# visinf/style-seqcvae

Hardware: AMD Instinct MI355X
Metric: captions/sec (train step) (higher is better)
Workload: dtype f32; 1 GPU; C2 train step: fwd+bwd+allreduce+clip+SGD, B=64/GPU, R=36, F=2048, L=20 (T=21), Z=128, V=10000, E=1000, H=1200, A=768, SENTIMENT_VAE=1; global_batch=64, parallelism=dp1

## Files before the change

style-seqcvae_amd/csrc/gemm.hip:

```cpp
#include <stdio.h>
#include <stdlib.h>
#include <string.h>

#include <type_traits>

#include "ssc_common.h"
#include "ssc_debug.h"

typedef float f32x16 __attribute__((ext_vector_type(16)));

namespace {

constexpr int BM = 64, BN = 64, BK = 32;
constexpr int KC_LD = BK + 4;

struct KSeg {
  const float* A;
  const float* B;
  int lda, ldb, K, nsteps;
  int avec, bvec;
  const float* A16;
  const float* B16;
  int lda16, ldb16;
};
// ... 829 lines not shown
      SSC_X3B_MFMA(1, 1)
      SSC_X3B_MFMA(1, 0)
      SSC_X3B_MFMA(0, 1)
      SSC_X3B_MFMA(0, 0)
#undef SSC_X3B_MFMA
    }
  };

  for (int s = s_lo; s < s_hi; ++s) {
    compute();
    wait_loads();
    __syncthreads();
    if (s + 1 < s_hi) put_planes();
    advance();
    issue_loads();
    __syncthreads();
  }
  wait_loads();

  float* out = a.out + (size_t)z * a.slab_stride;
#pragma unroll
  for (int ni = 0; ni < 2; ++ni) {
    const int col = n0 + wn * 64 + ni * 32 + l31;
    if (col >= a.N) continue;
    const float bv = (a.bias != nullptr) ? a.bias[col] : 0.f;
#pragma unroll
    for (int mi = 0; mi < 2; ++mi) {
      const int rbase = m0 + wm * 64 + mi * 32 + 4 * half;
      int rr[16];
#pragma unroll
      for (int r = 0; r < 16; ++r) {
        rr[r] = min(rbase + (r & 3) + 8 * (r >> 2), Meff - 1);
        if (a.crows) rr[r] = a.crows[rr[r]];
      }
      float old[16];
      if (a.accumulate) {
#pragma unroll
        for (int r = 0; r < 16; ++r) old[r] = out[(size_t)rr[r] * a.ldo + col];
      } else {
#pragma unroll
        for (int r = 0; r < 16; ++r) old[r] = 0.f;
      }
#pragma unroll
      for (int r = 0; r < 16; ++r) {
        if (rbase + (r & 3) + 8 * (r >> 2) < Meff) out[(size_t)rr[r] * a.ldo + col] = acc[mi][ni][r] + bv + old[r];
      }
    }
  }
}


#ifdef SSC_X3W_STAMP
__device__ unsigned long long* g_stamp_ptr = nullptr;
__device__ int g_stamp_wg = -1;
#define SSC_STAMP(i)                                                                                  \
  do {                                                                                                \
    if (stamp_on && lane == 0 && (i) < 124) stamp_lds[(i)] = __builtin_readcyclecounter();           \
  } while (0)
constexpr int X3W_STAMP_BYTES = 2048;
#else
#define SSC_STAMP(i) do {} while (0)
constexpr int X3W_STAMP_BYTES = 0;
#endif
#ifdef SSC_X3W_AUDIT
constexpr int SSC_AUDIT_MEMBERS = 20;
__device__ long long g_audit[SSC_AUDIT_MEMBERS][SSC_MAX_SEG][2][2];
#define SSC_AUDIT_TOUCH(member, seg, op, off)                                       \
  do {                                                                              \
    atomicMin(&g_audit[(member)][(seg)][(op)][0], (long long)(off));                \
    atomicMax(&g_audit[(member)][(seg)][(op)][1], (long long)(off) + 16);           \
  } while (0)
#else
#define SSC_AUDIT_TOUCH(member, seg, op, off) do {} while (0)
#endif
template <int R> struct X3wPlane {
  static constexpr int MC_ROW_B = 2 * R + 64;
  static constexpr int KC_BYTES = R * PL_ROW_B, MC_BYTES = 32 * MC_ROW_B;
  static constexpr int BYTES = KC_BYTES > MC_BYTES ? KC_BYTES : MC_BYTES;
};
template <int TM, int TN> constexpr int x3w_lds_bytes() { return 2 * 3 * (X3wPlane<TM>::BYTES + X3wPlane<TN>::BYTES) + X3W_STAMP_BYTES; }
template <int TM, int TN> constexpr int x3w_lds_bytes_f16() { return 2 * 2 * (X3wPlane<TM>::BYTES + X3wPlane<TN>::BYTES) + X3W_STAMP_BYTES; }

struct KTnArgs;
template <bool A_KC, bool B_KC, bool KG, int TM, int TN, int PF, int NPW, bool F16 = false, class Args = KArgs>
__device__ __forceinline__ void x3w_body(const Args& a, const int blk_x, const int blk_y, const int blk_z, const int grid_x,
                                         const int grid_y, const int grid_z, const int thr) {
  static_assert((TM == 128 && TN == 128) || (TM == 64 && TN == 256), "unsupported tile");
  static_assert(PF == 1 || PF == 2, "prefetch depth");
  constexpr int UNR = 2;
  constexpr bool RL = TM == 128;
  static_assert(!KG || PF == 1, "the gather lists' own loads share the vector-memory counter");
  constexpr int NPL = F16 ? 2 : 3;
  constexpr int PLA = X3wPlane<TM>::BYTES, PLB = X3wPlane<TN>::BYTES, STAGE = NPL * (PLA + PLB);
  static_assert(TM * (TN + 4) * 4 <= 2 * STAGE, "the epilogue's C tile reuses the operand stages");
  constexpr int MCA = X3wPlane<TM>::MC_ROW_B, MCB = X3wPlane<TN>::MC_ROW_B;
  static_assert(NPW == 4 || NPW == 8, "producer waves");
  constexpr int NPT = 64 * NPW;
  constexpr int NTHR = 256 + NPT;
  constexpr int NA = TM * 8 / NPT, NB = TN * 8 / NPT;
  constexpr int QA = TM / 4, QB = TN / 4;
  auto kc_row = [&](int t, int u, int) __attribute__((always_inline)) -> int { return (t + NPT * u) >> 3; };
  extern __shared__ __attribute__((aligned(16))) unsigned char lds[];
  const int wave = thr >> 6;
  const bool producer = wave >= 4;
  const int tid = producer ? thr - 256 : thr;
  const int lane = tid & 63;
  int bx, by;
  const int Meff = (RL && a.mcount) ? min(a.M, *a.mcount) : a.M;
  const int gy_live = min(grid_y, (Meff + TM - 1) / TM);
  if (blk_y * grid_x + blk_x >= grid_x * gy_live) return;
  tile_order(blk_y * grid_x + blk_x, grid_x, gy_live, a.tile_gm, bx, by);
  const int n0 = bx * TN, m0 = by * TM, z = blk_z;
  if (m0 >= Meff) return;
  const int Kc = a.kcount ? max(0, min(a.seg[0].K, *a.kcount)) : 0;
  int steps_total = a.steps_total, steps_per_split = a.steps_per_split;
  if (a.kcount) {
    steps_total = (Kc + BK - 1) / BK;
    steps_per_split = (steps_total + grid_z - 1) / grid_z;
  }
  const int s_lo = z * steps_per_split;
  int s_hi = s_lo + steps_per_split;
  if (s_hi > steps_total) s_hi = steps_total;
  const int s_last = s_hi - 1;
  constexpr int CT_LD = TN + 4;
  float f16_sa = 1.f, f16_sb = 1.f;
  if constexpr (F16) {
    if (a.a_scale) f16_sa = *a.a_scale;
    if (a.b_scale) f16_sb = *a.b_scale;
  }
#ifdef SSC_X3W_STAMP
  const bool stamp_on = (int)blockIdx.x == g_stamp_wg && (wave == 0 || wave == 4);
  unsigned long long* stamp_lds = reinterpret_cast<unsigned long long*>(lds + 2 * STAGE) + (wave == 4 ? 0 : 128);
  if (stamp_on && lane == 0) { stamp_lds[126] = __builtin_readcyclecounter(); stamp_lds[127] = wall_clock64(); }
  const unsigned long long stamp_entry = wall_clock64();
#endif

  if (producer) {
    f32x4 ra[PF][NA], rb[PF][NB];
    unsigned oka[PF], okb[PF];
    bool fullk[PF];
    unsigned oa[NA], ob[NB];
    unsigned za[NA], zb[NB];
    int ia[2][NA], ib[2][NB];
    Cursor cur;
    int s_ld = s_lo;
    bool pa = false, pb = false;
    auto planes_of_segment = [&]() __attribute__((always_inline)) {
      if constexpr (F16) {
        const KSeg& sg = a.seg[cur.seg];
        pa = sg.A16 != nullptr; pb = sg.B16 != nullptr;
        if (pa) { cur.A = sg.A16; cur.lda = sg.lda16; }
        if (pb) { cur.B = sg.B16; cur.ldb = sg.ldb16; }
      }
    };
    auto base_ptrs = [&]() __attribute__((always_inline)) {
      const unsigned lda4 = (unsigned)cur.lda * 4u, ldb4 = (unsigned)cur.ldb * 4u;
#pragma unroll
      for (int u = 0; u < NA; ++u) {
        const int idx = tid + NPT * u;
        if constexpr (A_KC) {
          int r = min(m0 + kc_row(tid, u, NA), Meff - 1);
          if constexpr (RL) { if (a.arows) r = a.arows[r]; }
          za[u] = (unsigned)r * lda4;
          oa[u] = za[u] + 16u * (idx & 7);
        } else {
          za[u] = 4u * (unsigned)min(m0 + 4 * (idx % QA), Meff - 4);
          if constexpr (KG) {
            int kr = cur.k0 + idx / QA;
            kr = a.karows[min(kr, cur.K - 1)];
            oa[u] = (unsigned)kr;
          } else {
            oa[u] = (unsigned)(idx / QA) * lda4 + za[u];
          }
        }
      }
#pragma unroll
      for (int u = 0; u < NB; ++u) {
        const int idx = tid + NPT * u;
        if constexpr (B_KC) {
          zb[u] = (unsigned)min(n0 + kc_row(tid, u, NB), a.N - 1) * ldb4;
          ob[u] = zb[u] + 16u * (idx & 7);
        } else {
          zb[u] = 4u * (unsigned)min(n0 + 4 * (idx % QB), a.N - 4);
          if constexpr (KG) {
            int kr = cur.k0 + idx / QB;
            kr = a.kbrows[min(kr, cur.K - 1)];
            ob[u] = (unsigned)kr;
          } else {
            ob[u] = (unsigned)(idx / QB) * ldb4 + zb[u];
          }
        }
      }
    };
    auto prefetch_rows = [&](int buf) __attribute__((always_inline)) {
      if constexpr (KG) {
#pragma unroll
        for (int u = 0; u < NA; ++u) {
          const int kr = min(cur.k0 + BK + (tid + NPT * u) / QA, cur.K - 1);
          ia[buf][u] = a.karows[kr];
        }
#pragma unroll
        for (int u = 0; u < NB; ++u) {
          const int kr = min(cur.k0 + BK + (tid + NPT * u) / QB, cur.K - 1);
          ib[buf][u] = a.kbrows[kr];
        }
      }
    };
    auto step_ptrs = [&](int how, int buf) __attribute__((always_inline)) {
      if constexpr (KG) {
        if (how != 0) {
#pragma unroll
          for (int u = 0; u < NA; ++u) oa[u] = (unsigned)ia[buf][u];
#pragma unroll
          for (int u = 0; u < NB; ++u) ob[u] = (unsigned)ib[buf][u];
          prefetch_rows(buf ^ 1);
        }
      } else {
        if (how == 2) base_ptrs();
      }
    };
    auto issue_loads = [&](f32x4 (&xa)[NA], f32x4 (&xb)[NB], unsigned& ma, unsigned& mb, bool& full) __attribute__((always_inline)) {
      ma = pa ? 0x80000000u : 0u;
      mb = pb ? 0x80000000u : 0u;
      full = cur.k0 + BK <= cur.K;
      const float* sa = cur.A + (A_KC ? (size_t)cur.k0 : (KG ? (size_t)0 : (size_t)cur.k0 * cur.lda));
      const float* sb = cur.B + (B_KC ? (size_t)cur.k0 : (KG ? (size_t)0 : (size_t)cur.k0 * cur.ldb));
      unsigned ea[NA], eb[NB];
      const bool kc_in = cur.k0 + 4 * (tid & 7) < cur.K;
#pragma unroll
      for (int u = 0; u < NA; ++u) {
        const int idx = tid + NPT * u;
        if constexpr (A_KC) {
          ea[u] = (kc_in || pa) ? oa[u] : za[u];
          ma |= (kc_in ? 1u : 0u) << u;
        } else {
          const bool in = cur.k0 + idx / QA < cur.K;
          if constexpr (KG) ea[u] = __umul24(oa[u], (unsigned)cur.lda * 4u) + za[u];
          else ea[u] = in ? oa[u] : za[u];
          ma |= (in ? 1u : 0u) << u;
        }
      }
#pragma unroll
      for (int u = 0; u < NB; ++u) {
        const int idx = tid + NPT * u;
        if constexpr (B_KC) {
          eb[u] = (kc_in || pb) ? ob[u] : zb[u];
          mb |= (kc_in ? 1u : 0u) << u;
        } else {
          const bool in = cur.k0 + idx / QB < cur.K;
          if constexpr (KG) eb[u] = __umul24(ob[u], (unsigned)cur.ldb * 4u) + zb[u];
          else eb[u] = in ? ob[u] : zb[u];
          mb |= (in ? 1u : 0u) << u;
        }
      }
#ifdef SSC_X3W_AUDIT
#pragma unroll
      for (int u = 0; u < NA; ++u) SSC_AUDIT_TOUCH(a.member, cur.seg, 0, (reinterpret_cast<const char*>(sa) - reinterpret_cast<const char*>(cur.A)) + (long long)ea[u]);
#pragma unroll
      for (int u = 0; u < NB; ++u) SSC_AUDIT_TOUCH(a.member, cur.seg, 1, (reinterpret_cast<const char*>(sb) - reinterpret_cast<const char*>(cur.B)) + (long long)eb[u]);
#endif
#pragma unroll
      for (int u = 0; u < NA; ++u) asm volatile("global_load_dwordx4 %0, %1, %2" : "=&v"(xa[u]) : "v"(ea[u]), "s"(sa) : "memory");
#pragma unroll
      for (int u = 0; u < NB; ++u) asm volatile("global_load_dwordx4 %0, %1, %2" : "=&v"(xb[u]) : "v"(eb[u]), "s"(sb) : "memory");
    };
    auto pin = [&](f32x4 (&xa)[NA], f32x4 (&xb)[NB]) __attribute__((always_inline)) {
#pragma unroll
      for (int u = 0; u < NA; ++u) asm volatile("" : "+v"(xa[u])::"memory");
#pragma unroll
      for (int u = 0; u < NB; ++u) asm volatile("" : "+v"(xb[u])::"memory");
    };
    auto advance = [&](int buf) __attribute__((always_inline)) {
      const int how = cur.advance(a, s_ld >= s_last);
      s_ld = min(s_ld + 1, s_last);
      if (how == 2) planes_of_segment();
      step_ptrs(how, buf);
    };
    auto put_chunk = [&](unsigned char* p, int plane, f32x4 v, bool ok, float scale) __attribute__((always_inline)) {
      if (!ok) v = f32x4{0.f, 0.f, 0.f, 0.f};
      if constexpr (F16) {
        u32x2 hi, lo;
        v = v * scale;
        split4_f16(v, hi, lo);
        *reinterpret_cast<u32x2*>(p) = hi;
        *reinterpret_cast<u32x2*>(p + plane) = lo;
      } else {
        u32x2 hi, mid, lo;
// ... 299 lines not shown
        const float e[4] = {v.x, v.y, v.z, v.w};
#pragma unroll
        for (int q = 0; q < 4; ++q) {
          if (gcol + q < a.N) {
            const float r = e[q] + (a.bias ? a.bias[gcol + q] : 0.f) + (a.accumulate ? dst[q] : 0.f);
            dst[q] = r;
            if constexpr (std::is_same_v<Args, KTnArgs>) {
              if (a.out2) a.out2[(size_t)grow * a.ldo2 + gcol + q] = r;
            }
          }
        }
      }
    }
  }
#ifdef SSC_X3W_STAMP
  if (stamp_on && lane == 0) { stamp_lds[124] = __builtin_readcyclecounter(); stamp_lds[125] = wall_clock64(); }
  __syncthreads();
  if ((int)blockIdx.x == g_stamp_wg && thr < 256 && g_stamp_ptr)
    g_stamp_ptr[thr] = reinterpret_cast<const unsigned long long*>(lds + 2 * STAGE)[thr];
  if (g_stamp_wg == -2 && thr == 0 && g_stamp_ptr && blockIdx.x < 1024) {
    g_stamp_ptr[2 * blockIdx.x] = stamp_entry;
    g_stamp_ptr[2 * blockIdx.x + 1] = wall_clock64();
  }
#endif
}


constexpr int SSC_GROUP_MAX = 6;
struct KGroup {
  KArgs a[SSC_GROUP_MAX];
  int n;
  int first[SSC_GROUP_MAX + 1];
  int gx[SSC_GROUP_MAX], gy[SSC_GROUP_MAX], gz[SSC_GROUP_MAX];
};
template <bool A_KC, bool B_KC, bool KG, int TM, int TN, int PF, int NPW, bool F16 = false>
__global__ __launch_bounds__(256 + 64 * NPW, (F16 && NPW == 4) ? 4 : 1) void gemm_x3w_kernel(const KGroup g) {
  const int w = blockIdx.x;
  int p = 0;
#pragma unroll
  for (int i = 1; i < SSC_GROUP_MAX; ++i)
    if (i < g.n && w >= g.first[i]) p = i;
  const int local = w - g.first[p];
  const int gx = g.gx[p], gy = g.gy[p], gz = g.gz[p];
  const int x = local % gx, yz = local / gx;
  x3w_body<A_KC, B_KC, KG, TM, TN, PF, NPW, F16>(g.a[p], x, yz % gy, yz / gy, gx, gy, gz, (int)threadIdx.x);
}

constexpr int SSC_DW_MAX = 20;
struct KTnMember {
  const float* A;
  const float* B;
  float* C;
  const int* kcount;
  const int* karows;
  const int* kbrows;
  int lda, ldb, ldc, M, N, K, accumulate;
  int first;
  float* C2;
  int ldc2;
};
struct KTnList {
  KTnMember m[SSC_DW_MAX];
  int n, total;
  int tile_gm, store_wt;
};
struct KOneSeg {
  KSeg s;
  __device__ __forceinline__ const KSeg& operator[](int) const { return s; }
};
struct KTnArgs {
  KOneSeg seg;
  int nseg, M, N;
  float* out;
  int ldo;
  size_t slab_stride;
  const float* bias;
  int accumulate, steps_total, steps_per_split;
  const int *mcount, *arows, *crows, *kcount, *karows, *kbrows;
  int tile_gm, store_wt, member;
  float* topk;
  const float *a_scale, *b_scale;
  float* out2;
  int ldo2;
};
template <int PF, int NPW>
__global__ __launch_bounds__(256 + 64 * NPW, 1) void gemm_x3w_kernel_tn_list(const KTnList g) {
  int p = 0;
  for (int t = blockIdx.x; t < g.total; t += gridDim.x) {
#pragma unroll 1
    while (p + 1 < g.n && t >= g.m[p + 1].first) ++p;
    const KTnMember& m = g.m[p];
    int thr = (int)threadIdx.x;
    asm volatile("" : "+v"(thr));
    __builtin_assume(thr >= 0 && thr < 256 + 64 * NPW);
    KTnArgs a;
    a.seg.s.A = m.A; a.seg.s.B = m.B; a.seg.s.lda = m.lda; a.seg.s.ldb = m.ldb; a.seg.s.K = m.K;
    a.seg.s.nsteps = (m.K + BK - 1) / BK; a.seg.s.avec = a.seg.s.bvec = 1;
    a.seg.s.A16 = a.seg.s.B16 = nullptr; a.seg.s.lda16 = a.seg.s.ldb16 = 0;
    a.nseg = 1; a.M = m.M; a.N = m.N;
    a.out = m.C; a.ldo = m.ldc; a.slab_stride = 0; a.bias = nullptr; a.accumulate = m.accumulate;
    a.steps_total = a.steps_per_split = a.seg.s.nsteps;
    a.mcount = a.arows = a.crows = nullptr;
    a.kcount = m.kcount; a.karows = m.karows; a.kbrows = m.kbrows;
    a.tile_gm = g.tile_gm; a.store_wt = g.store_wt; a.member = p;
    a.topk = nullptr; a.a_scale = a.b_scale = nullptr;
    a.out2 = m.C2; a.ldo2 = m.ldc2;
    const int gx = (m.N + 127) / 128, gy = (m.M + 127) / 128;
    const int local = t - m.first;
    x3w_body<false, false, true, 128, 128, PF, NPW>(a, local % gx, local / gx, 0, gx, gy, 1, thr);
    __syncthreads();
  }
}

__global__ void reduce_slabs_kernel(const float* __restrict__ slabs, int nslab, size_t slab_stride, int M, int N,
                                    float* __restrict__ C, int ldc, const float* __restrict__ bias, int accumulate,
                                    const int* __restrict__ mcount, const int* __restrict__ crows) {
  size_t i = (size_t)blockIdx.x * blockDim.x + threadIdx.x;
  if (mcount) M = min(M, *mcount);
  size_t total = (size_t)M * N;
  if (i >= total) return;
  int row = (int)(i / N), col = (int)(i % N);
  float v = 0.f;
  for (int s0 = 0; s0 < nslab; s0 += 8) {
    float t[8];
#pragma unroll
    for (int u = 0; u < 8; ++u) t[u] = slabs[(size_t)min(s0 + u, nslab - 1) * slab_stride + i];
#pragma unroll
    for (int u = 0; u < 8; ++u) v += (s0 + u < nslab) ? t[u] : 0.f;
  }
  if (bias) v += bias[col];
  if (crows) row = crows[row];
  float* p = C + (size_t)row * ldc + col;
  if (accumulate) v += *p;
  *p = v;
}

typedef void (*gemm_fn)(const KArgs);

struct ProfMember { int M, N, K, slot_m, slot_k; };
struct ProfRec {
  hipEvent_t e0, e1;
  int kind, M, N, K, splits;
  double bytes, flops;
  ProfMember mem[8];
  int nmem;
};
int* g_prof_counts = nullptr;
int g_prof_slots = 0;
constexpr int PROF_SLOTS = 8192;
inline int prof_count_slot(const int* dev_count, hipStream_t st) {
  if (!dev_count || !g_prof_counts || g_prof_slots >= PROF_SLOTS) return -1;
  const int slot = g_prof_slots++;
  g_prof_counts[slot] = -1;
  if (hipMemcpyAsync(&g_prof_counts[slot], dev_count, sizeof(int), hipMemcpyDeviceToHost, st) != hipSuccess) return -1;
  return slot;
}
inline void prof_desc(ProfRec* rec, const ssc_gemm_desc* d, hipStream_t st) {
  int K = 0;
  for (int i = 0; i < d->nseg; ++i) K += d->seg[i].K;
  if (rec->nmem < 8) {
    ProfMember& m = rec->mem[rec->nmem++];
    m.M = d->M; m.N = d->N; m.K = K;
    m.slot_m = prof_count_slot(d->m_count, st);
    m.slot_k = prof_count_slot(d->k_count, st);
  }
}
constexpr int PROF_MAX = 4096;
ProfRec* g_prof = nullptr;
int g_prof_n = 0;
bool g_prof_on = false;

int g_store_wt = ssc_env_int("SSC_STORE_WT", 1);
int g_tile_gm = ssc_env_int("SSC_TILE_GM", 8);
int build_args(const ssc_gemm_desc* d, KArgs& k) {
  if (!d || d->nseg < 1 || d->nseg > SSC_MAX_SEG || d->M <= 0 || d->N <= 0) return SSC_EINVAL;
  k.tile_gm = g_tile_gm;
  k.store_wt = g_store_wt;
  k.member = 0;
  k.nseg = d->nseg;
  k.M = d->M;
  k.N = d->N;
  k.mcount = d->m_count; k.arows = d->a_rows; k.crows = d->c_rows;
  k.kcount = d->k_count; k.karows = d->ka_rows; k.kbrows = d->kb_rows;
  k.a_scale = d->a_scale; k.b_scale = d->b_scale;
  k.topk = d->topk_part;
  k.steps_total = 0;
  for (int i = 0; i < d->nseg; ++i) {
    const ssc_gemm_seg& s = d->seg[i];
    if (!s.A || !s.B || s.K <= 0) return SSC_EINVAL;
    int min_lda = d->a_kc ? s.K : d->M, min_ldb = d->b_kc ? s.K : d->N;
    if (s.lda < min_lda || s.ldb < min_ldb) return SSC_EINVAL;
    if ((((uintptr_t)s.A) & 3u) || (((uintptr_t)s.B) & 3u)) return SSC_EALIGN;
// ... 64 lines not shown
  (void)hipMemcpyToSymbol(HIP_SYMBOL(g_audit), init, sizeof(init));
}
long audit_rows(const int* list, const int* count, int nominal) {
  int n = nominal;
  if (count) { (void)hipMemcpy(&n, count, sizeof(int), hipMemcpyDeviceToHost); if (n > nominal) n = nominal; if (n < 0) n = 0; }
  if (!list) return n;
  if (n == 0) return 0;
  int* h = (int*)malloc((size_t)n * sizeof(int));
  (void)hipMemcpy(h, list, (size_t)n * sizeof(int), hipMemcpyDeviceToHost);
  long mx = 0;
  for (int i = 0; i < n; ++i) if (h[i] + 1 > mx) mx = h[i] + 1;
  free(h);
  return mx;
}
void audit_end(const KArgs* ka, int n, bool a_kc, bool b_kc, const char* what, hipStream_t st) {
  (void)hipStreamSynchronize(st);
  long long got[SSC_AUDIT_MEMBERS][SSC_MAX_SEG][2][2];
  (void)hipMemcpyFromSymbol(got, HIP_SYMBOL(g_audit), sizeof(got));
  ++g_audit_launches;
  for (int m = 0; m < n; ++m) {
    const KArgs& k = ka[m];
    for (int sg = 0; sg < k.nseg; ++sg) {
      const long K = k.kcount ? audit_rows(nullptr, k.kcount, k.seg[sg].K) : k.seg[sg].K;
      for (int op = 0; op < 2; ++op) {
        const long long lo = got[m][sg][op][0], hi = got[m][sg][op][1];
        if (hi <= lo) continue;
        const bool kc = op == 0 ? a_kc : b_kc;
        const long ld = op == 0 ? k.seg[sg].lda : k.seg[sg].ldb;
        const long width = op == 0 ? k.M : k.N;
        long long span;
        if (kc) {
          const long rows = op == 0 ? audit_rows(k.arows, k.mcount, k.M) : width;
          span = rows > 0 ? ((long long)(rows - 1) * ld + k.seg[sg].K) * 4 : 0;
        } else {
          const long krows = audit_rows(op == 0 ? k.karows : k.kbrows, k.kcount, k.seg[sg].K);
          span = krows > 0 ? ((long long)(krows - 1) * ld + width) * 4 : (long long)width * 4;
        }
        (void)K;
        ++g_audit_records;
        if (lo < 0 || hi > span) {
          ++g_audit_violations;
          fprintf(stderr, "[x3w audit] VIOLATION %s member %d segment %d operand %c: touched bytes [%lld, %lld) of a span of %lld (M %d N %d K %d ld %ld)\n",
                  what, m, sg, op == 0 ? 'A' : 'B', lo, hi, span, k.M, k.N, k.seg[sg].K, ld);
        }
      }
    }
  }
}
#define SSC_AUDIT_BEGIN() audit_begin()
#define SSC_AUDIT_END(ka, n, a_kc, b_kc, what, st) audit_end(ka, n, a_kc, b_kc, what, st)
#else
#define SSC_AUDIT_BEGIN() do {} while (0)
#define SSC_AUDIT_END(ka, n, a_kc, b_kc, what, st) do {} while (0)
#endif
inline void group_of_one(KGroup& g, const KArgs& k, dim3 grid) {
  g.a[0] = k;
  g.a[0].member = 0;
  g.n = 1;
  g.first[0] = 0;
  for (int i = 0; i < SSC_GROUP_MAX; ++i) {
    g.first[i + 1] = (int)(grid.x * grid.y * grid.z);
    g.gx[i] = (int)grid.x; g.gy[i] = (int)grid.y; g.gz[i] = (int)grid.z;
  }
}

struct X3wForm { group_fn fn; int threads, lds; const char* what; };
template <bool A_KC, bool B_KC, bool KG, int TM, int TN, int PF, int NPW, bool F16 = false>
constexpr X3wForm x3w_form(const char* what) {
  return {gemm_x3w_kernel<A_KC, B_KC, KG, TM, TN, PF, NPW, F16>, 256 + 64 * NPW, F16 ? x3w_lds_bytes_f16<TM, TN>() : x3w_lds_bytes<TM, TN>(), what};
}
enum { X3W_NT, X3W_NN, X3W_TN, X3W_TN_KG, X3W_NT_F16_4, X3W_NT_F16_8, X3W_SKINNY_NT, X3W_SKINNY_NN, X3W_FORMS };
const X3wForm g_x3w[X3W_FORMS] = {
    x3w_form<true, true, false, 128, 128, 2, 8>("128x128"), x3w_form<true, false, false, 128, 128, 2, 8>("128x128"),
    x3w_form<false, false, false, 128, 128, 2, 8>("128x128"), x3w_form<false, false, true, 128, 128, 1, 8>("128x128"),
    x3w_form<true, true, false, 128, 128, 2, 4, true>("128x128 f16"), x3w_form<true, true, false, 128, 128, 2, 8, true>("128x128 f16"),
    x3w_form<true, true, false, 64, 256, 2, 8>("64x256"), x3w_form<true, false, false, 64, 256, 2, 8>("64x256"),
};
inline const X3wForm& x3w_big(bool a_kc, bool b_kc, bool kg) {
  return g_x3w[(a_kc && b_kc) ? X3W_NT : a_kc ? X3W_NN : kg ? X3W_TN_KG : X3W_TN];
}
inline const X3wForm& x3w_skinny_form(bool b_kc) { return g_x3w[b_kc ? X3W_SKINNY_NT : X3W_SKINNY_NN]; }

typedef void (*tn_list_fn)(const KTnList);
const tn_list_fn g_tn_list_fn = gemm_x3w_kernel_tn_list<1, 8>;
constexpr int TN_LIST_THREADS = 256 + 64 * 8, TN_LIST_LDS = x3w_lds_bytes<128, 128>();
int g_cus[64] = {};

int x3w_prepare() {
  static bool done_dev[64] = {};
  int dev = 0;
  if (hipGetDevice(&dev) != hipSuccess || dev < 0 || dev >= 64) return SSC_EHIP;
  bool& done = done_dev[dev];
  if (done) return SSC_OK;
  for (const X3wForm& f : g_x3w)
    if (hipFuncSetAttribute((const void*)f.fn, hipFuncAttributeMaxDynamicSharedMemorySize, f.lds) != hipSuccess) return SSC_EHIP;
  if (hipFuncSetAttribute((const void*)g_tn_list_fn, hipFuncAttributeMaxDynamicSharedMemorySize, TN_LIST_LDS) != hipSuccess) return SSC_EHIP;
  if (hipDeviceGetAttribute(&g_cus[dev], hipDeviceAttributeMultiprocessorCount, dev) != hipSuccess || g_cus[dev] < 1) return SSC_EHIP;
  done = true;
  return SSC_OK;
}

inline bool x3w_span_ok(const ssc_gemm_desc* d) {
  const size_t lim = (size_t)1 << 30;
  if (d->ka_rows || d->kb_rows)
    for (int i = 0; i < d->nseg; ++i)
      if (d->seg[i].lda >= (1 << 22) || d->seg[i].ldb >= (1 << 22) || d->seg[i].K >= (1 << 24)) return false;
  for (int i = 0; i < d->nseg; ++i) {
    const size_t K = (size_t)d->seg[i].K;
    if (K == 0) continue;
    const size_t sa = d->a_kc ? (size_t)(d->M - 1) * d->seg[i].lda + K : (K - 1) * d->seg[i].lda + d->M;
    const size_t sb = d->b_kc ? (size_t)(d->N - 1) * d->seg[i].ldb + K : (K - 1) * d->seg[i].ldb + d->N;
    if (sa >= lim || sb >= lim) return false;
    const size_t kp = (K + BK - 1) / BK * BK;
    if (d->seg[i].A16 && (size_t)(d->M - 1) * d->seg[i].lda16 + kp >= lim) return false;
    if (d->seg[i].B16 && (size_t)(d->N - 1) * d->seg[i].ldb16 + kp >= lim) return false;
  }
  return true;
}
inline bool vec_all(const KArgs& k) {
  for (int i = 0; i < k.nseg; ++i)
    if (!k.seg[i].avec || !k.seg[i].bvec) return false;
  return true;
}
inline bool x3w_ok(const ssc_gemm_desc* d, const KArgs& k, Num num) {
  return num != Num::F32 && vec_all(k) && (d->a_kc || !d->b_kc) && x3w_span_ok(d);
}

struct Form {
  gemm_fn fn = nullptr;
  const X3wForm* x3w = nullptr;
  dim3 grid;
};
int plan(const ssc_gemm_desc* d, const KArgs& k, int splits, Num num, Form& f) {
  const bool x3 = num != Num::F32, vec = vec_all(k);
  const bool mlist = k.mcount || k.arows || k.crows, klist = k.kcount || k.karows || k.kbrows;
  const bool compact = mlist || klist;
  if (k.topk && !(x3 && vec && d->a_kc && d->b_kc && splits == 1 && !klist && x3w_span_ok(d))) return SSC_EINVAL;
  if (compact) {
    if (!vec) return SSC_EALIGN;
    if (!x3 || (!d->a_kc && d->b_kc)) return SSC_EINVAL;
    if (klist && (k.nseg != 1 || d->a_kc || d->b_kc)) return SSC_EINVAL;
    if (mlist && !d->a_kc) return SSC_EINVAL;
  }
  if (!compact && !k.topk && x3w_skinny_layout(d) && x3w_skinny_shape(d->M, d->N, num) && x3w_ok(d, k, num)) {
    f.x3w = &x3w_skinny_form(d->b_kc);
    f.grid = dim3(ssc_cdiv(d->N, 256), ssc_cdiv(d->M, 64), splits);
    return SSC_OK;
  }
  if (x3 && vec && (d->a_kc || !d->b_kc) && (compact || k.topk || (g_x3b && big_tile(d->M, d->N)))) {
    f.grid = dim3(ssc_cdiv(d->N, 128), ssc_cdiv(d->M, 128), splits);
    const bool kg = k.karows || k.kbrows;
    const long wgs = (long)f.grid.x * f.grid.y * f.grid.z;
    const bool f16 = num == Num::X3_F16 && d->a_kc && d->b_kc && !kg && g_x3b != 3;
    const bool x3w = k.topk || g_x3b == 2 || (g_x3b == 1 && (f16 || wgs >= 768 || (d->M < 512 && big_tile(d->M, d->N))));
    if (x3w && x3w_span_ok(d) && (!kg || (k.karows && k.kbrows))) {
      f.x3w = f16 ? &g_x3w[g_f16_npw == 4 ? X3W_NT_F16_4 : X3W_NT_F16_8] : &x3w_big(d->a_kc, d->b_kc, kg);
      return SSC_OK;
    }
    f.fn = (d->a_kc && d->b_kc) ? gemm_x3b_kernel<true, true, false>
           : d->a_kc            ? gemm_x3b_kernel<true, false, false>
           : kg                 ? gemm_x3b_kernel<false, false, true>
                                : gemm_x3b_kernel<false, false, false>;
    return SSC_OK;
  }
  if (x3 && vec && d->a_kc && d->b_kc) {
    f.fn = gemm_x3_kernel;
    f.grid = dim3(ssc_cdiv(d->N, 64), ssc_cdiv(d->M, 64), splits);
    return SSC_OK;
  }
  const bool big = big_tile(d->M, d->N);
  const bool wide = !big && vec && wide_tile(d->M, d->N);
  f.grid = dim3(ssc_cdiv(d->N, (big || wide) ? 128 : 64), ssc_cdiv(d->M, big ? 128 : 64), splits);
  f.fn = big ? (vec ? pick_layout<2, 2, 1, true>(d) : pick_layout<2, 2, 1, false>(d))
             : wide ? pick_layout<1, 2, 2, true>(d)
                    : (vec ? pick_layout<1, 1, 4, true>(d) : pick_layout<1, 1, 2, false>(d));
  return SSC_OK;
}

ProfRec* prof_open(const ssc_gemm_desc* const* d, int n, int M, int N, int K, int splits, hipStream_t st) {
// ... 117 lines not shown
    if (!np[g]) continue;
    part[g].nseg = np[g];
    int ksteps = 0;
    for (int i = 0; i < np[g]; ++i) ksteps += ssc_cdiv(part[g].seg[i].K, BK);
    int splits = ssc_gemm_auto_splits(d->M, d->N, ksteps);
    if (d->m_count || d->a_rows || d->c_rows) splits = 1;
    while (splits > 1 && (size_t)(total + splits) * mn > cap_floats) --splits;
    if ((size_t)(total + splits) * mn > cap_floats) return SSC_EWORKSPACE;
    int per = ssc_cdiv(ksteps, splits);
    splits = ssc_cdiv(ksteps, per);
    SSC_TRY(ssc_gemm_slabs(&part[g], splits, slabs + (size_t)total * mn, st));
    total += splits;
  }
  *nslab = total;
  return SSC_OK;
}

int ssc_gemm_slabs_group(const ssc_gemm_desc* const* d, int n, float* const* regions, const size_t* caps, int* nslab,
                         hipStream_t st) {
  if (!d || n < 1 || n > SSC_GROUP_MAX || !regions || !caps || !nslab) return SSC_EINVAL;
  const Num num = numerics();
  KGroup g;
  bool ok = n >= 2, any_wide = false;
  long work = 0;
  const bool mid = d[0] && d[0]->M > 64 && d[0]->M >= BIG_MIN_M;
  const int tw = mid ? 128 : 256;
  for (int i = 0; i < n && ok; ++i) {
    SSC_TRY(build_args(d[i], g.a[i]));
    const KArgs& k = g.a[i];
    const bool compact = k.mcount || k.arows || k.crows || k.kcount || k.karows || k.kbrows;
    const bool shape = mid ? g_x3b != 0 && g_x3b != 3 && d[i]->M >= BIG_MIN_M && d[i]->M < 512 && d[i]->M == d[0]->M
                           : x3w_skinny_layout(d[i]) && d[i]->M <= 64;
    ok = !compact && x3w_ok(d[i], k, num) && d[i]->a_kc && shape && d[i]->N >= 64 && d[i]->b_kc == d[0]->b_kc && regions[i];
    any_wide = any_wide || (mid ? big_tile(d[i]->M, d[i]->N) : d[i]->N >= X3W_MIN_N);
    work += (long)ssc_cdiv(d[i]->N, tw) * ssc_cdiv(d[i]->M, mid ? 128 : 64) * k.steps_total;
  }
  ok = ok && any_wide;
  if (!ok) {
    for (int i = 0; i < n; ++i) SSC_TRY(ssc_gemm_slabs_auto(d[i], regions[i], caps[i], &nslab[i], st));
    return SSC_OK;
  }
  int per = (int)((work + 255) / 256);
  if (per < 4) per = 4;
  for (;; ++per) {
    long wgs = 0;
    for (int i = 0; i < n; ++i) wgs += (long)ssc_cdiv(d[i]->N, tw) * ssc_cdiv(d[i]->M, mid ? 128 : 64) * ssc_cdiv(g.a[i].steps_total, per);
    if (wgs <= 256 || per >= 4096) break;
  }
  g.n = n;
  g.first[0] = 0;
  int Ksum = 0, Nmax = 0;
  for (int i = 0; i < n; ++i) {
    KArgs& k = g.a[i];
    k.member = i;
    const size_t mn = (size_t)d[i]->M * d[i]->N;
    int splits = ssc_cdiv(k.steps_total, per);
    const int cap = (int)(caps[i] / mn);
    if (cap < 1) return SSC_EWORKSPACE;
    if (splits > cap) splits = cap;
    const int p2 = ssc_cdiv(k.steps_total, splits);
    splits = ssc_cdiv(k.steps_total, p2);
    k.steps_per_split = p2;
    k.out = regions[i];
    k.ldo = d[i]->N;
    k.slab_stride = mn;
    k.bias = nullptr;
    k.accumulate = 0;
    k.crows = nullptr;
    g.gx[i] = ssc_cdiv(d[i]->N, tw);
    g.gy[i] = mid ? ssc_cdiv(d[i]->M, 128) : 1;
    g.gz[i] = splits;
    g.first[i + 1] = g.first[i] + g.gx[i] * g.gy[i] * splits;
    nslab[i] = splits;
    for (int s = 0; s < d[i]->nseg; ++s) Ksum += d[i]->seg[s].K;
    if (d[i]->N > Nmax) Nmax = d[i]->N;
  }
  for (int i = n; i < SSC_GROUP_MAX; ++i) { g.first[i + 1] = g.first[n]; g.gx[i] = 1; g.gy[i] = 1; g.gz[i] = 1; }
  ProfRec* rec = prof_open(d, n, d[0]->M, Nmax, Ksum, nslab[0], st);
  if (mid) return launch_x3w(x3w_big(true, d[0]->b_kc != 0, false), g, true, d[0]->b_kc != 0, "128x128 group", rec, st);
  return launch_x3w(x3w_skinny_form(d[0]->b_kc != 0), g, true, d[0]->b_kc != 0, "64x256 group", rec, st);
}

namespace {
int launch_tn_list(const ssc_gemm_desc* const* d, const KArgs* ka, int n, hipStream_t st) {
  SSC_TRY(x3w_prepare());
  int dev = 0;
  if (hipGetDevice(&dev) != hipSuccess) return SSC_EHIP;
  int ord[SSC_DW_MAX];
  for (int i = 0; i < n; ++i) ord[i] = i;
  for (int i = 1; i < n; ++i)
    for (int j = i; j > 0 && ka[ord[j]].steps_total > ka[ord[j - 1]].steps_total; --j) { const int t = ord[j]; ord[j] = ord[j - 1]; ord[j - 1] = t; }
  KTnList g;
  memset(&g, 0, sizeof(g));
  const ssc_gemm_desc* ds[SSC_DW_MAX];
  KArgs audit[SSC_DW_MAX];
  int first = 0;
  long MN = 0;
  for (int i = 0; i < n; ++i) {
    const ssc_gemm_desc* di = d[ord[i]];
    KTnMember& m = g.m[i];
    m.A = di->seg[0].A; m.B = di->seg[0].B; m.C = di->C;
    m.kcount = di->k_count; m.karows = di->ka_rows; m.kbrows = di->kb_rows;
    m.lda = di->seg[0].lda; m.ldb = di->seg[0].ldb; m.ldc = di->ldc;
    m.M = di->M; m.N = di->N; m.K = di->seg[0].K; m.accumulate = di->accumulate;
    m.C2 = di->C2; m.ldc2 = di->ldc2;
    m.first = first;
    first += ssc_cdiv(di->M, 128) * ssc_cdiv(di->N, 128);
    MN += (long)di->M * di->N;
    ds[i] = di;
    audit[i] = ka[ord[i]];
    audit[i].out = di->C; audit[i].ldo = di->ldc;
  }
  g.n = n; g.total = first;
  g.tile_gm = g_tile_gm; g.store_wt = g_store_wt;
  ProfRec* rec = prof_open(ds, n, (int)(MN / ds[0]->N), ds[0]->N, ds[0]->seg[0].K, 1, st);
  SSC_AUDIT_BEGIN();
  SSC_LAUNCH(g_tn_list_fn, dim3(first < g_cus[dev] ? first : g_cus[dev]), dim3(TN_LIST_THREADS), TN_LIST_LDS, st, g);
  SSC_AUDIT_END(audit, n, false, false, "128x128 TN list", st);
  (void)audit;
  prof_close(rec, st);
  SSC_CHECK_LAUNCH();
  return SSC_OK;
}
}
extern "C" int ssc_gemm_dw_group(const ssc_gemm_desc* const* d, int n, void* stream) {
  hipStream_t st = (hipStream_t)stream;
  constexpr int NMAX = 32;
  if (!d || n < 1 || n > NMAX) return SSC_EINVAL;
  const Num num = numerics();
  KArgs ka[NMAX];
  int cls[NMAX];
  for (int j = 0; j < n; ++j) {
    const ssc_gemm_desc* dj = d[j];
    KArgs& k = ka[j];
    SSC_TRY(build_args(dj, k));
    if (dj->C2 && (dj->ldc2 < dj->N || !dj->C)) return SSC_EINVAL;
    const bool kg = k.karows || k.kbrows;
    const bool ok = x3w_ok(dj, k, num) && k.nseg == 1 && !dj->a_kc && !dj->b_kc && dj->C && dj->ldc >= dj->N && !k.mcount &&
                    !k.arows && !k.crows && (kg ? (k.kcount && k.karows && k.kbrows && !dj->bias) : !k.kcount);
    cls[j] = !ok ? 0 : kg ? 2 : 1;
  }
  const ssc_gemm_desc* ld[SSC_DW_MAX];
  KArgs lk[SSC_DW_MAX];
  int ln = 0;
  for (int j = 0; j < n; ++j) {
    if (cls[j] != 2) continue;
    ld[ln] = d[j]; lk[ln] = ka[j];
    if (++ln == SSC_DW_MAX) { SSC_TRY(launch_tn_list(ld, lk, ln, st)); ln = 0; }
  }
  if (ln) SSC_TRY(launch_tn_list(ld, lk, ln, st));
  int i = 0;
  while (i < n) {
    if (cls[i] == 2) { ++i; continue; }
    int m = 0;
    while (cls[i] == 1 && i + m < n && cls[i + m] == 1 && m < SSC_GROUP_MAX) ++m;
    if (m >= 2) {
      KGroup g;
      g.n = m;
      g.first[0] = 0;
      long MN = 0;
      for (int q = 0; q < m; ++q) {
        const ssc_gemm_desc* dj = d[i + q];
        KArgs& k = g.a[q];
        k = ka[i + q];
        k.member = q;
        k.steps_per_split = k.steps_total;
        k.out = dj->C; k.ldo = dj->ldc; k.slab_stride = 0; k.bias = dj->bias; k.accumulate = dj->accumulate;
        g.gx[q] = ssc_cdiv(dj->N, 128); g.gy[q] = ssc_cdiv(dj->M, 128); g.gz[q] = 1;
        g.first[q + 1] = g.first[q] + g.gx[q] * g.gy[q];
        MN += (long)dj->M * dj->N;
      }
      for (int q = m; q < SSC_GROUP_MAX; ++q) { g.first[q + 1] = g.first[m]; g.gx[q] = g.gy[q] = g.gz[q] = 1; }
      ProfRec* rec = prof_open(d + i, m, (int)(MN / d[i]->N), d[i]->N, d[i + m - 1]->seg[0].K, 1, st);
      SSC_TRY(launch_x3w(x3w_big(false, false, false), g, false, false, "128x128 TN group", rec, st));
      i += m;
    } else {
      ssc_gemm_desc one = *d[i];
      one.C2 = nullptr;
      SSC_TRY(ssc_gemm(&one, (void*)st));
      ++i;
    }
  }
  for (int j = 0; j < n; ++j)
    if (d[j]->C2 && cls[j] != 2 &&
        hipMemcpy2DAsync(d[j]->C2, (size_t)d[j]->ldc2 * sizeof(float), d[j]->C, (size_t)d[j]->ldc * sizeof(float),
                         (size_t)d[j]->N * sizeof(float), d[j]->M, hipMemcpyDeviceToDevice, st) != hipSuccess)
      return SSC_EHIP;
  return SSC_OK;
}

namespace {
__global__ __launch_bounds__(256) void split_f16_kernel(const float* __restrict__ x, int rows, int K, int ldx, const float* __restrict__ scale,
                                                        unsigned* __restrict__ out, int ldo, const int* __restrict__ row_list,
                                                        const int* __restrict__ row_count) {
  const int kq = blockIdx.x * blockDim.x + threadIdx.x;
  const int kp4 = (K + BK - 1) / BK * (BK / 4);
  if (kq >= kp4) return;
  const float sc = scale ? *scale : 1.f;
  const int n = row_list ? min(rows, *row_count) : rows;
  const bool vec = !(ldx & 3) && ssc_aligned16_dev(x);
  const int k = 4 * kq;
  for (int i = blockIdx.y; i < n; i += gridDim.y) {
    const int r = row_list ? row_list[i] : i;
    const float* xr = x + (size_t)r * ldx;
// ... 44 lines not shown
    splits = d->workspace ? (int)(d->workspace_floats / ((size_t)d->M * d->N)) : 1;
    if (splits < 1) splits = 1;
    int per = ssc_cdiv(k.steps_total, splits);
    splits = ssc_cdiv(k.steps_total, per);
  }
  if (splits == 1) {
    k.out = d->C;
    k.ldo = d->ldc;
    k.slab_stride = 0;
    k.bias = d->bias;
    k.accumulate = d->accumulate;
    return launch(d, k, 1, st);
  }
  k.out = d->workspace;
  k.ldo = d->N;
  k.slab_stride = (size_t)d->M * d->N;
  k.bias = nullptr;
  k.accumulate = 0;
  k.crows = nullptr;
  SSC_TRY(launch(d, k, splits, st));
  size_t total = (size_t)d->M * d->N;
  SSC_LAUNCH(reduce_slabs_kernel, dim3((unsigned)((total + 255) / 256)), dim3(256), 0, st, d->workspace, splits,
                     k.slab_stride, d->M, d->N, d->C, d->ldc, d->bias, d->accumulate, d->m_count, d->c_rows);
  SSC_CHECK_LAUNCH();
  return SSC_OK;
}

extern "C" int ssc_prof_enable(int on) {
  if (on && !g_prof) {
    g_prof = new ProfRec[PROF_MAX];
    for (int i = 0; i < PROF_MAX; ++i) {
      if (hipEventCreate(&g_prof[i].e0) != hipSuccess || hipEventCreate(&g_prof[i].e1) != hipSuccess) return SSC_EHIP;
    }
  }
  if (on && !g_prof_counts && hipHostMalloc((void**)&g_prof_counts, PROF_SLOTS * sizeof(int), hipHostMallocDefault) != hipSuccess) return SSC_EHIP;
  g_prof_on = on != 0;
  if (on) { g_prof_n = 0; g_prof_slots = 0; }
  return SSC_OK;
}

extern "C" int ssc_prof_collect(float* out, int max_records) {
  if (!out || !g_prof) return 0;
  if (hipDeviceSynchronize() != hipSuccess) return SSC_EHIP;
  int n = g_prof_n < max_records ? g_prof_n : max_records;
  for (int i = 0; i < n; ++i) {
    float ms = 0.f;
    (void)hipEventElapsedTime(&ms, g_prof[i].e0, g_prof[i].e1);
    float* o = out + (size_t)i * 8;
    g_prof[i].bytes = g_prof[i].flops = 0.0;
    for (int q = 0; q < g_prof[i].nmem; ++q) {
      const ProfMember& m = g_prof[i].mem[q];
      double M = m.M, K = m.K;
      if (m.slot_m >= 0 && g_prof_counts[m.slot_m] >= 0 && g_prof_counts[m.slot_m] < m.M) M = g_prof_counts[m.slot_m];
      if (m.slot_k >= 0 && g_prof_counts[m.slot_k] >= 0 && g_prof_counts[m.slot_k] < m.K) K = g_prof_counts[m.slot_k];
      g_prof[i].bytes += 4.0 * (K * m.N + M * K + M * m.N);
      g_prof[i].flops += 2.0 * M * m.N * K;
    }
    o[0] = (float)g_prof[i].kind; o[1] = (float)g_prof[i].M; o[2] = (float)g_prof[i].N; o[3] = (float)g_prof[i].K;
    o[4] = (float)g_prof[i].splits; o[5] = ms; o[6] = (float)g_prof[i].bytes; o[7] = (float)g_prof[i].flops;
  }
  g_prof_n = 0;
  g_prof_slots = 0;
  return n;
}

extern "C" int ssc_set_gemm_mode(int mode) {
  int prev = gemm_mode();
  if (mode == 0 || mode == 1) g_gemm_mode = mode;
  return prev;
}

extern int ssc_g_dec_att_table, ssc_g_dec_dedup, ssc_g_beam_reg, ssc_g_dec_ungathered, ssc_g_dec_parts, ssc_g_dec_planes;
extern int ssc_g_img_mfma;
extern int ssc_g_dw_one_flush;
extern int ssc_g_stream_nt;
namespace {
struct DebugKey { const char* name; int* var; };
const DebugKey g_debug_keys[] = {
    {"large_form", &g_x3b},
    {"x3w_skinny", &g_x3w_skinny},
    {"store_wt", &g_store_wt},
    {"tile_gm", &g_tile_gm},
    {"dw_one_flush", &ssc_g_dw_one_flush},
    {"dec_dedup", &ssc_g_dec_dedup},
    {"beam_reg", &ssc_g_beam_reg},
    {"img_mfma", &ssc_g_img_mfma},
    {"dec_ungathered", &ssc_g_dec_ungathered},
    {"dec_planes", &ssc_g_dec_planes},
    {"dec_parts", &ssc_g_dec_parts},
    {"dec_att_table", &ssc_g_dec_att_table},
    {"f16_npw", &g_f16_npw},
    {"stream_nt", &ssc_g_stream_nt},
    {"gemm_f16", &g_gemm_f16},
};
}

extern "C" int ssc_debug_set(const char* key, int value) {
  if (!key) return SSC_EINVAL;
  for (const DebugKey& k : g_debug_keys)
    if (!strcmp(k.name, key)) { *k.var = value; return SSC_OK; }
  return SSC_EINVAL;
}
extern "C" int ssc_debug_get(const char* key, int* value) {
  if (!key || !value) return SSC_EINVAL;
  for (const DebugKey& k : g_debug_keys)
    if (!strcmp(k.name, key)) { *value = *k.var; return SSC_OK; }
  return SSC_EINVAL;
}

#ifdef SSC_X3W_STAMP
extern "C" int ssc_debug_stamp_setup(void* buf, int wg) {
  if (hipMemcpyToSymbol(HIP_SYMBOL(g_stamp_ptr), &buf, sizeof(buf)) != hipSuccess) return SSC_EHIP;
  if (hipMemcpyToSymbol(HIP_SYMBOL(g_stamp_wg), &wg, sizeof(wg)) != hipSuccess) return SSC_EHIP;
  return SSC_OK;
}
#endif
```

Baseline: 8055 captions/s.

## Stage gather row lists in LDS to enable double-buffered prefetch in TN list GEMM

The weight-gradient TN work-list kernel gets a variant that copies the k-gather row index lists into LDS whenever the member changes. Its row lookups then read LDS instead of global memory, so the lists no longer compete on the vector-memory counter and the kernel can run with prefetch depth 2. Members whose K fits in the LDS list budget go to this variant by default, the rest stay on the old path. This costs extra LDS, an added sync per member switch, and a possible second launch. An optional grid cap knob is also added.

Result: no change. 8121 captions/s, median of 6 (+0.8%).

```diff
diff --git a/style-seqcvae_amd/csrc/gemm.hip b/style-seqcvae_amd/csrc/gemm.hip
--- a/style-seqcvae_amd/csrc/gemm.hip
+++ b/style-seqcvae_amd/csrc/gemm.hip
@@ -935,14 +935,16 @@
 template <int TM, int TN> constexpr int x3w_lds_bytes_f16() { return 2 * 2 * (X3wPlane<TM>::BYTES + X3wPlane<TN>::BYTES) + X3W_STAMP_BYTES; }
 
 struct KTnArgs;
-template <bool A_KC, bool B_KC, bool KG, int TM, int TN, int PF, int NPW, bool F16 = false, class Args = KArgs>
+constexpr int X3W_LIST_INTS = 9728;
+template <bool A_KC, bool B_KC, bool KG, int TM, int TN, int PF, int NPW, bool F16 = false, class Args = KArgs, bool KL = false>
 __device__ __forceinline__ void x3w_body(const Args& a, const int blk_x, const int blk_y, const int blk_z, const int grid_x,
                                          const int grid_y, const int grid_z, const int thr) {
   static_assert((TM == 128 && TN == 128) || (TM == 64 && TN == 256), "unsupported tile");
   static_assert(PF == 1 || PF == 2, "prefetch depth");
   constexpr int UNR = 2;
   constexpr bool RL = TM == 128;
-  static_assert(!KG || PF == 1, "the gather lists' own loads share the vector-memory counter");
+  static_assert(!KG || PF == 1 || KL, "gather lists in global memory: their loads share the vector-memory counter, PF == 1");
+  static_assert(!KL || (KG && std::is_same_v<Args, KTnArgs>), "LDS lists: the work-list form");
   constexpr int NPL = F16 ? 2 : 3;
   constexpr int PLA = X3wPlane<TM>::BYTES, PLB = X3wPlane<TN>::BYTES, STAGE = NPL * (PLA + PLB);
   static_assert(TM * (TN + 4) * 4 <= 2 * STAGE, "the epilogue's C tile reuses the operand stages");
@@ -965,7 +967,12 @@
   tile_order(blk_y * grid_x + blk_x, grid_x, gy_live, a.tile_gm, bx, by);
   const int n0 = bx * TN, m0 = by * TM, z = blk_z;
   if (m0 >= Meff) return;
-  const int Kc = a.kcount ? max(0, min(a.seg[0].K, *a.kcount)) : 0;
+  int Kc;
+  if constexpr (KL) Kc = a.kc;
+  else Kc = a.kcount ? max(0, min(a.seg[0].K, *a.kcount)) : 0;
+  [[maybe_unused]] const int* lrows_a = reinterpret_cast<const int*>(lds + 2 * STAGE + X3W_STAMP_BYTES);
+  [[maybe_unused]] const int* lrows_b = lrows_a;
+  if constexpr (KL) lrows_b = lrows_a + a.lrows_b;
   int steps_total = a.steps_total, steps_per_split = a.steps_per_split;
   if (a.kcount) {
     steps_total = (Kc + BK - 1) / BK;
@@ -1020,7 +1027,8 @@
           za[u] = 4u * (unsigned)min(m0 + 4 * (idx % QA), Meff - 4);
           if constexpr (KG) {
             int kr = cur.k0 + idx / QA;
-            kr = a.karows[min(kr, cur.K - 1)];
+            if constexpr (KL) kr = lrows_a[min(kr, cur.K - 1)];
+            else kr = a.karows[min(kr, cur.K - 1)];
             oa[u] = (unsigned)kr;
           } else {
             oa[u] = (unsigned)(idx / QA) * lda4 + za[u];
@@ -1037,7 +1045,8 @@
           zb[u] = 4u * (unsigned)min(n0 + 4 * (idx % QB), a.N - 4);
           if constexpr (KG) {
             int kr = cur.k0 + idx / QB;
-            kr = a.kbrows[min(kr, cur.K - 1)];
+            if constexpr (KL) kr = lrows_b[min(kr, cur.K - 1)];
+            else kr = a.kbrows[min(kr, cur.K - 1)];
             ob[u] = (unsigned)kr;
           } else {
             ob[u] = (unsigned)(idx / QB) * ldb4 + zb[u];
@@ -1050,12 +1059,14 @@
 #pragma unroll
         for (int u = 0; u < NA; ++u) {
           const int kr = min(cur.k0 + BK + (tid + NPT * u) / QA, cur.K - 1);
-          ia[buf][u] = a.karows[kr];
+          if constexpr (KL) ia[buf][u] = lrows_a[kr];
+          else ia[buf][u] = a.karows[kr];
         }
 #pragma unroll
         for (int u = 0; u < NB; ++u) {
           const int kr = min(cur.k0 + BK + (tid + NPT * u) / QB, cur.K - 1);
-          ib[buf][u] = a.kbrows[kr];
+          if constexpr (KL) ib[buf][u] = lrows_b[kr];
+          else ib[buf][u] = a.kbrows[kr];
         }
       }
     };
@@ -1521,14 +1532,32 @@
   const float *a_scale, *b_scale;
   float* out2;
   int ldo2;
+  int kc, lrows_b;
 };
-template <int PF, int NPW>
+template <int PF, int NPW, bool KL>
 __global__ __launch_bounds__(256 + 64 * NPW, 1) void gemm_x3w_kernel_tn_list(const KTnList g) {
   int p = 0;
+  [[maybe_unused]] const int *c_kc = nullptr, *c_ka = nullptr, *c_kb = nullptr;
+  [[maybe_unused]] int c_K = -1, c_live = 0;
   for (int t = blockIdx.x; t < g.total; t += gridDim.x) {
 #pragma unroll 1
     while (p + 1 < g.n && t >= g.m[p + 1].first) ++p;
     const KTnMember& m = g.m[p];
+    if constexpr (KL) {
+      if (m.kcount != c_kc || m.karows != c_ka || m.kbrows != c_kb || m.K != c_K) {
+        extern __shared__ __attribute__((aligned(16))) unsigned char lds_raw[];
+        int* la = reinterpret_cast<int*>(lds_raw + x3w_lds_bytes<128, 128>());
+        c_kc = m.kcount; c_ka = m.karows; c_kb = m.kbrows; c_K = m.K;
+        c_live = max(0, min(m.K, *m.kcount));
+        const bool one = m.karows == m.kbrows;
+        int* lb = la + (one ? 0 : X3W_LIST_INTS / 2);
+        for (int i = (int)threadIdx.x; i < c_live; i += 256 + 64 * NPW) {
+          la[i] = m.karows[i];
+          if (!one) lb[i] = m.kbrows[i];
+        }
+        __syncthreads();
+      }
+    }
     int thr = (int)threadIdx.x;
     asm volatile("" : "+v"(thr));
     __builtin_assume(thr >= 0 && thr < 256 + 64 * NPW);
@@ -1544,9 +1573,10 @@
     a.tile_gm = g.tile_gm; a.store_wt = g.store_wt; a.member = p;
     a.topk = nullptr; a.a_scale = a.b_scale = nullptr;
     a.out2 = m.C2; a.ldo2 = m.ldc2;
+    a.kc = c_live; a.lrows_b = m.karows == m.kbrows ? 0 : X3W_LIST_INTS / 2;
     const int gx = (m.N + 127) / 128, gy = (m.M + 127) / 128;
     const int local = t - m.first;
-    x3w_body<false, false, true, 128, 128, PF, NPW>(a, local % gx, local / gx, 0, gx, gy, 1, thr);
+    x3w_body<false, false, true, 128, 128, PF, NPW, false, KTnArgs, KL>(a, local % gx, local / gx, 0, gx, gy, 1, thr);
     __syncthreads();
   }
 }
@@ -1777,8 +1807,13 @@
 inline const X3wForm& x3w_skinny_form(bool b_kc) { return g_x3w[b_kc ? X3W_SKINNY_NT : X3W_SKINNY_NN]; }
 
 typedef void (*tn_list_fn)(const KTnList);
-const tn_list_fn g_tn_list_fn = gemm_x3w_kernel_tn_list<1, 8>;
-constexpr int TN_LIST_THREADS = 256 + 64 * 8, TN_LIST_LDS = x3w_lds_bytes<128, 128>();
+const tn_list_fn g_tn_list_fn[2] = {gemm_x3w_kernel_tn_list<1, 8, false>, gemm_x3w_kernel_tn_list<2, 8, true>};
+constexpr int TN_LIST_THREADS = 256 + 64 * 8;
+constexpr int TN_LIST_LDS[2] = {x3w_lds_bytes<128, 128>(), x3w_lds_bytes<128, 128>() + X3W_LIST_INTS * 4};
+static_assert(TN_LIST_LDS[1] <= 160 * 1024, "LDS of a compute unit");
+int g_dw_pf = ssc_env_int("SSC_DW_PF", 2);
+int g_dw_grid = ssc_env_int("SSC_DW_GRID", 0);
+inline bool tn_list_fits(const ssc_gemm_desc* d) { return d->seg[0].K <= (d->ka_rows == d->kb_rows ? X3W_LIST_INTS : X3W_LIST_INTS / 2); }
 int g_cus[64] = {};
 
 int x3w_prepare() {
@@ -1789,7 +1824,8 @@
   if (done) return SSC_OK;
   for (const X3wForm& f : g_x3w)
     if (hipFuncSetAttribute((const void*)f.fn, hipFuncAttributeMaxDynamicSharedMemorySize, f.lds) != hipSuccess) return SSC_EHIP;
-  if (hipFuncSetAttribute((const void*)g_tn_list_fn, hipFuncAttributeMaxDynamicSharedMemorySize, TN_LIST_LDS) != hipSuccess) return SSC_EHIP;
+  for (int i = 0; i < 2; ++i)
+    if (hipFuncSetAttribute((const void*)g_tn_list_fn[i], hipFuncAttributeMaxDynamicSharedMemorySize, TN_LIST_LDS[i]) != hipSuccess) return SSC_EHIP;
   if (hipDeviceGetAttribute(&g_cus[dev], hipDeviceAttributeMultiprocessorCount, dev) != hipSuccess || g_cus[dev] < 1) return SSC_EHIP;
   done = true;
   return SSC_OK;
@@ -2073,7 +2109,7 @@
 }
 
 namespace {
-int launch_tn_list(const ssc_gemm_desc* const* d, const KArgs* ka, int n, hipStream_t st) {
+int launch_tn_list_form(const ssc_gemm_desc* const* d, const KArgs* ka, int n, bool lds_lists, hipStream_t st) {
   SSC_TRY(x3w_prepare());
   int dev = 0;
   if (hipGetDevice(&dev) != hipSuccess) return SSC_EHIP;
@@ -2106,11 +2142,24 @@
   g.tile_gm = g_tile_gm; g.store_wt = g_store_wt;
   ProfRec* rec = prof_open(ds, n, (int)(MN / ds[0]->N), ds[0]->N, ds[0]->seg[0].K, 1, st);
   SSC_AUDIT_BEGIN();
-  SSC_LAUNCH(g_tn_list_fn, dim3(first < g_cus[dev] ? first : g_cus[dev]), dim3(TN_LIST_THREADS), TN_LIST_LDS, st, g);
+  int grid = first < g_cus[dev] ? first : g_cus[dev];
+  if (g_dw_grid > 0 && grid > g_dw_grid) grid = g_dw_grid;
+  SSC_LAUNCH(g_tn_list_fn[lds_lists ? 1 : 0], dim3(grid), dim3(TN_LIST_THREADS), TN_LIST_LDS[lds_lists ? 1 : 0], st, g);
   SSC_AUDIT_END(audit, n, false, false, "128x128 TN list", st);
   (void)audit;
   prof_close(rec, st);
   SSC_CHECK_LAUNCH();
+  return SSC_OK;
+}
+int launch_tn_list(const ssc_gemm_desc* const* d, const KArgs* ka, int n, hipStream_t st) {
+  const ssc_gemm_desc* sd[SSC_DW_MAX];
+  KArgs sk[SSC_DW_MAX];
+  for (int pass = 0; pass < 2; ++pass) {
+    int sn = 0;
+    for (int i = 0; i < n; ++i)
+      if ((g_dw_pf != 1 && tn_list_fits(d[i])) == (pass == 0)) { sd[sn] = d[i]; sk[sn] = ka[i]; ++sn; }
+    if (sn) SSC_TRY(launch_tn_list_form(sd, sk, sn, pass == 0, st));
+  }
   return SSC_OK;
 }
 }
@@ -2321,6 +2370,8 @@
     {"store_wt", &g_store_wt},
     {"tile_gm", &g_tile_gm},
     {"dw_one_flush", &ssc_g_dw_one_flush},
+    {"dw_pf", &g_dw_pf},
+    {"dw_grid", &g_dw_grid},
     {"dec_dedup", &ssc_g_dec_dedup},
     {"beam_reg", &ssc_g_beam_reg},
     {"img_mfma", &ssc_g_img_mfma},
```
